# MasterXiong/Hyper-VLA

Hardware: AMD Instinct MI355X
Metric: actions_per_sec (higher is better)
Workload: dtype f16; 1 GPU; BASELINE configs[1]: hypernet weight-gen once (untimed) + full sample_actions step (u8 224x224 -> DINOv2-base E=768 in the loop -> generated vit_t 4L/64d policy -> [4,7] action chunk); 1 action = 1 sample-step; batch_per_gpu=256, global_batch=256, encoder=DINOv2-base (reference parity, E=768), parallelism=episode-dp1 (no collectives), policy_operands=split-bf16 (bf16x3), launch=eager (114 launches per step, counted by the library), streams=1, ensemble=not in the step

## Files before the change

hyper-vla_amd/csrc/api.hip:

```cpp
#include <hip/hip_runtime.h>

#include <cmath>
#include <cstdio>
#include <cstring>
#include <map>
#include <memory>
#include <mutex>
#include <string>
#include <vector>

#include "../../include/hvla.h"
#include "common.h"
#include "kernels.h"
#include "layout.h"
#include "pack.h"
#include "t5.h"
#include "train.h"

using namespace hvla;

namespace {

struct DevBuf {
  void* p = nullptr;
// ... 23 lines not shown
  int B = 0, H = 0;
  DevBuf ring;
  DevBuf state;
};

struct hvla_ctx {
  hvla_config cfg{};
  Geom g{};
  int device = 0;
  std::string err;
  bool loaded = false;
  bool train_timer = false;
  PackedLayout lay;
  int Kp = 0;
  DevBuf hn_f32;
  CtxParams ctxp{};
  DevBuf wcat_hi, wcat_lo, bcat, perm;
  DevBuf enc16, encd16, encf32;
  EncWeights encw{};
  DevBuf ctx_hi, ctx_lo, ctx_f32, ws_x, ws_h, ws_qkv, ws_g, ws_corr, ws_abar, ws_lncnt, ws_lnpart, tokens, flags;
  uint32_t ln_spin = 800;
#ifdef HVLA_BENCH_HOOKS
  int enc_stop = 0;
#endif
  Profiler prof;
  float *amap_dino = nullptr, *amap_head = nullptr;
  hipStream_t side = nullptr;
  hipEvent_t ev_fork = nullptr, ev_join = nullptr;
  std::vector<hvla_weights*> arena_pool;
  std::mutex pool_mu;
  static constexpr size_t ARENA_POOL_MAX = 4;
  hipEvent_t ev_bucket[3] = {nullptr, nullptr, nullptr};
  bool bucket_recorded[3] = {false, false, false};
  ~hvla_ctx() {
    for (hvla_weights* w : arena_pool) delete w;
    for (hipEvent_t e : ev_bucket)
      if (e) (void)hipEventDestroy(e);
    if (ev_fork) (void)hipEventDestroy(ev_fork);
    if (ev_join) (void)hipEventDestroy(ev_join);
    if (side) (void)hipStreamDestroy(side);
  }
  int rs_H = 0, rs_W = 0, rs_row_span = 0, rs_col_span = 0;
  DevBuf rs_tab, rs_rows, rs_img, rs_pad;
  bool t5_loaded = false;
  T5Dims t5d{};
  T5Weights t5w{};
// ... 406 lines not shown
  return HVLA_OK;
}

static int check_step(hvla_ctx* ctx, int32_t B) {
  if (!ctx->loaded) FAIL(ctx, HVLA_E_STATE, "called before hvla_load_weights");
  if (B < 1 || B > ctx->cfg.max_batch) FAIL(ctx, HVLA_E_SHAPE, "batch %d outside [1, %d]", B, ctx->cfg.max_batch);
  return HVLA_OK;
}

static int encode_range(hvla_ctx* ctx, const uint8_t* images, float* out, int b0, int nb, bool keep_cls, hipStream_t st) {
  const Geom& g = ctx->g;
  const size_t S = g.S(), E = g.E, F = g.enc_mlp, rows = (size_t)b0 * S;
  const size_t gper = S * F > (size_t)g.P() * ctx->Kp ? S * F : (size_t)g.P() * ctx->Kp;
  EncWorkspace ws{ctx->ws_x.as<float>() + rows * E, static_cast<char*>(ctx->ws_h.p) + rows * E * 2,
                  static_cast<char*>(ctx->ws_qkv.p) + rows * 3 * E * 2, static_cast<char*>(ctx->ws_g.p) + (size_t)b0 * gper * 2,
                  ctx->ws_corr.as<float>() + (size_t)2 * b0 * (F > 3 * E ? F : 3 * E),
                  static_cast<char*>(ctx->ws_abar.p) + (size_t)2 * b0 * (F > E ? F : E) * 2};
  if (ctx->amap_dino) ws.amap = ctx->amap_dino + (size_t)b0 * g.enc_layers * g.enc_heads * g.P();
  ws.ln_cnt = ctx->ws_lncnt.as<uint32_t>() + (size_t)((b0 + 3) / 4 * 4);
  ws.ln_part = ctx->ws_lnpart.as<float>() + (size_t)b0 * 4 * 256 * 4;
  ws.ln_spin = ctx->ln_spin;
#ifdef HVLA_BENCH_HOOKS
  ws.stop_after = ctx->enc_stop;
#endif
  const size_t img = (size_t)g.image_size * g.image_size * 3, per = (keep_cls ? S : (size_t)g.P()) * E;
  HIPCHK(ctx, launch_encoder(g, ctx->cfg.enc_dtype, ctx->encw, ws, images + (size_t)b0 * img, out + (size_t)b0 * per, nb, st,
                             &ctx->prof, keep_cls));
  return HVLA_OK;
}

int hvla_encode(hvla_ctx* ctx, const uint8_t* images, float* tokens, int32_t B, void* stream) {
  if (!ctx) return HVLA_E_STATE;
  if (int r = check_step(ctx, B)) return r;
  if (!images || !tokens) FAIL(ctx, HVLA_E_SHAPE, "null pointer");
  HIPCHK(ctx, hipSetDevice(ctx->device));
  return encode_range(ctx, images, tokens, 0, B, false, reinterpret_cast<hipStream_t>(stream));
}

int hvla_encode_hidden(hvla_ctx* ctx, const uint8_t* images, float* hidden, int32_t B, void* stream) {
  if (!ctx) return HVLA_E_STATE;
  if (int r = check_step(ctx, B)) return r;
  if (!images || !hidden) FAIL(ctx, HVLA_E_SHAPE, "null pointer");
  HIPCHK(ctx, hipSetDevice(ctx->device));
  return encode_range(ctx, images, hidden, 0, B, true, reinterpret_cast<hipStream_t>(stream));
}

// ... 619 lines not shown
  if (!ctx || !ptr || !bytes) return HVLA_E_STATE;
  DevBuf* b[8] = {&ctx->ws_x, &ctx->ws_h, &ctx->ws_qkv, &ctx->ws_g, &ctx->ws_corr, &ctx->ws_abar, &ctx->ws_lncnt, &ctx->ws_lnpart};
  if (which < 0 || which > 7) return HVLA_E_SHAPE;
  *ptr = b[which]->p;
  *bytes = b[which]->bytes;
  return HVLA_OK;
}
int hvla_debug_lnx_stats(hvla_ctx* ctx, unsigned long long* out, int reset) {
  if (!ctx) return HVLA_E_STATE;
  HIPCHK(ctx, hipSetDevice(ctx->device));
  HIPCHK(ctx, debug_lnx_stats(out, reset));
  return HVLA_OK;
}
int hvla_debug_encode_stop(hvla_ctx* ctx, int32_t n) {
  if (!ctx || n < 0) return HVLA_E_STATE;
  ctx->enc_stop = n;
  return HVLA_OK;
}
int hvla_debug_lnx_spin(hvla_ctx* ctx, uint32_t ticks) {
  if (!ctx) return HVLA_E_STATE;
  ctx->ln_spin = ticks;
  return HVLA_OK;
}
#endif

int64_t hvla_launches(hvla_ctx* ctx) {
  if (!ctx) return 0;
  const int64_t n = (int64_t)ctx->prof.nlaunch;
  ctx->prof.nlaunch = 0;
  return n;
}

int hvla_box_probe(hvla_ctx* ctx, float out[3], void* stream) {
  if (!ctx || !out) return HVLA_E_STATE;
  HIPCHK(ctx, hipSetDevice(ctx->device));
  DevBuf sink, ticks;
  int ncu = 256;
  (void)hipDeviceGetAttribute(&ncu, hipDeviceAttributeMultiprocessorCount, ctx->device);
  if (sink.alloc((size_t)ncu * 512 * sizeof(float)) != hipSuccess || ticks.alloc(64) != hipSuccess) FAIL(ctx, HVLA_E_ARENA_FULL, "box probe buffers");
  HIPCHK(ctx, run_box_probe(sink.as<float>(), ticks.as<unsigned long long>(), out, reinterpret_cast<hipStream_t>(stream)));
  return HVLA_OK;
}

int hvla_selftest(hvla_ctx* ctx, void* stream) {
  if (!ctx) return HVLA_E_STATE;
  HIPCHK(ctx, hipSetDevice(ctx->device));
// ... 13 lines not shown
```

hyper-vla_amd/csrc/encoder.hip:

```cpp
#include <cstring>
#include <type_traits>

#include "common.h"
#include "kernels.h"
#include "plan.h"

namespace hvla {

template <typename Op>
__global__ void im2col_kernel(const uint8_t* __restrict__ img, typename Op::elem* __restrict__ out, int B,
                              int image, int patch, int grid, int Kp, float* __restrict__ x, const float* __restrict__ pos, int S, int E) {
  for (size_t i = (size_t)blockIdx.x * blockDim.x + threadIdx.x; i < (size_t)B * E; i += (size_t)gridDim.x * blockDim.x)
    x[(i / E) * S * E + (i % E)] = pos[i % E];
  const int Kp1 = Kp / 2, chunks = Kp1 / 8;
  const size_t total = (size_t)B * grid * grid * chunks;
  const int kreal = patch * patch * 3;
  for (size_t i = (size_t)blockIdx.x * blockDim.x + threadIdx.x; i < total; i += (size_t)gridDim.x * blockDim.x) {
    const int ch = (int)(i % chunks);
    const size_t m = i / chunks;
    const int px = (int)(m % grid), py = (int)((m / grid) % grid);
    const size_t b = m / ((size_t)grid * grid);
    typename Op::x8 v;
    const int rowb = 3 * patch;
    const int k0 = ch * 8;
// ... 779 lines not shown
    reinterpret_cast<f32x4*>(partial + ((size_t)b * LNG + grp) * E)[threadIdx.x] = cs;
  }
}
template <typename Op>
__global__ __launch_bounds__(256) void layernorm_mean_kernel(const float* __restrict__ partial, typename Op::elem* __restrict__ abar,
                                                             int P, int E) {
  const int bh = blockIdx.x, n4 = E / 4;
  if ((int)threadIdx.x >= n4) return;
  const f32x4 t = ln_half_sum(reinterpret_cast<const f32x4*>(partial + (size_t)bh * 4 * E) + threadIdx.x, n4);
  const float inv = 1.f / (float)(P / 2);
  typename Op::x4 o;
#pragma unroll
  for (int j = 0; j < 4; ++j) o[j] = (typename Op::elem)(t[j] * inv);
  reinterpret_cast<typename Op::x4*>(abar + (size_t)bh * E)[threadIdx.x] = o;
}
constexpr int HBM_ = 256, HBN_ = 256;
constexpr int PRO_DMA = 12, PRO_DMA_KT0 = 8;
template <int EPI> struct EpiVmem { static constexpr int min_ops = (EPI == EPI_RES || EPI == EPI_PATCH) ? 64 : 32; };

#ifdef HVLA_BENCH_HOOKS
__device__ unsigned long long g_lnx_dbg[8][256];
#endif
constexpr int LNX_STAT = 98304, LNX_MR = LNX_STAT + 8192, LNX_CTRL = LNX_MR + 2048;
typedef __attribute__((address_space(3))) char lds_char;
template <typename Op, int EPI, bool PERSIST, bool LNX = false, bool NTOUT = false>
__global__ __launch_bounds__(512) void gemm256p_kernel(GemmArgs g) {
  static_assert(!NTOUT || EPI != EPI_PATCH, "NTOUT: non-temporal stores of the 16-bit outputs (QKV, GELU) / loads of the residual rows (RES)");
  using T = typename Op::elem;
  using X8 = typename Op::x8;
  static_assert(!LNX || EPI == EPI_RES || EPI == EPI_PATCH, "the fused LayerNorm follows a GEMM that writes the residual stream");
  extern __shared__ __attribute__((aligned(16))) char smem[];
  const int tid = threadIdx.x, lane = tid & 63;
  const int wave = __builtin_amdgcn_readfirstlane(tid >> 6);
  const int wm = wave >> 2, wn = wave & 3;
  const int nbm = g.nbm, nbn = (g.N + HBN_ - 1) / HBN_;
  const int ntiles = nbm * nbn;
  const int GN = nbn % 4 == 0 ? 4 : (nbn % 3 == 0 ? 3 : (nbn % 2 == 0 ? 2 : 1));
  auto tile_origin = [&](int v, int& tm, int& n0) {
    const int q = ntiles / 8, r = ntiles % 8, xcd = v % 8;
    const int bid = (xcd < r ? xcd * (q + 1) : r * (q + 1) + (xcd - r) * q) + v / 8;
    constexpr int CH = 8;
    const int per_chunk = CH * nbn;
    const int chunk = bid / per_chunk, rc = bid % per_chunk;
    const int rows = (nbm - chunk * CH) < CH ? (nbm - chunk * CH) : CH;
    const int sc = rc / (rows * GN), r2 = rc % (rows * GN);
    tm = chunk * CH + r2 / GN;
// ... 29 lines not shown
  const int sch = ((lane & 7) ^ (lane >> 3)) * 8;
  const uint32_t lane_a = ((uint32_t)srow * (uint32_t)g.K + sch) * (uint32_t)sizeof(T);
  const uint32_t lane_w = ((uint32_t)(wperm(srow)) * (uint32_t)g.K + sch) * (uint32_t)sizeof(T);
  const uint32_t lds0 = (uint32_t)(uintptr_t)(__attribute__((address_space(3))) char*)smem;
  const T* abase = A + (size_t)m0 * g.K;
  const T* wbase = W + (size_t)n0 * g.K;
  int wn0 = n0;
  const int KT = g.K / 64;
  auto stage = [&](auto hc, int kt) {
    constexpr int h = decltype(hc)::value;
    const int buf = kt & 1;
#pragma unroll
    for (int u = 0; u < 2; ++u) {
      const int j = 2 * (h & 1) + u;
      const int jw = (h < 2 || wn0 + 64 * j < g.N) ? j : 0;
      const T* sb = (h < 2 ? abase : wbase) + ((size_t)jw * 64 * g.K + kt * 64);
      const uint32_t dst = lds0 + (uint32_t)(buf * 65536 + wave * 1024 + (h >> 1) * 32768 + j * 8192);
      const uint32_t vo = h < 2 ? lane_a : lane_w;
      uint32_t keep;
      asm volatile("s_mov_b32 %0, m0\n\ts_mov_b32 m0, %3\n\ts_nop 0\n\tglobal_load_lds_dwordx4 %1, %2\n\ts_mov_b32 m0, %0"
                   : "=&s"(keep) : "v"(vo), "s"(sb), "s"(dst));
    }
  };
  f32x4 acc[4][8];
  const int fr = lane & 15, fq = lane >> 4;
  const int sw0 = ((fq) ^ (fr & 7)) << 4, sw1 = ((fq + 4) ^ (fr & 7)) << 4;
  const int a_off = (wm * 128 + fr) * 128, w_off = 32768 + (wn * 64 + fr) * 128;
  X8 fa0[8], fa1[8], fw0[4], fw1[4];
  auto rd_a = [&](X8 (&f)[8], const char* lb, int ah) {
#pragma unroll
    for (int t = 0; t < 4; ++t) {
      f[2 * t] = *reinterpret_cast<const X8*>(lb + a_off + (4 * ah + t) * 2048 + sw0);
      f[2 * t + 1] = *reinterpret_cast<const X8*>(lb + a_off + (4 * ah + t) * 2048 + sw1);
    }
  };
  auto rd_w = [&](X8 (&f)[4], const char* lb, int wh) {
#pragma unroll
    for (int t = 0; t < 2; ++t) {
      f[2 * t] = *reinterpret_cast<const X8*>(lb + w_off + (2 * wh + t) * 2048 + sw0);
      f[2 * t + 1] = *reinterpret_cast<const X8*>(lb + w_off + (2 * wh + t) * 2048 + sw1);
    }
  };
  auto quad = [&](const X8 (&fa)[8], const X8 (&fw)[4], auto ahc, auto whc) {
    constexpr int ah = decltype(ahc)::value, wh = decltype(whc)::value;
#pragma unroll
    for (int kk = 0; kk < 2; ++kk)
#pragma unroll
      for (int mt = 0; mt < 4; ++mt)
#pragma unroll
        for (int nt = 0; nt < 2; ++nt)
          acc[2 * wh + nt][4 * ah + mt] = Op::mma16(fa[2 * mt + kk], fw[2 * nt + kk], acc[2 * wh + nt][4 * ah + mt]);
  };
  using H0 = std::integral_constant<int, 0>;
  using H1 = std::integral_constant<int, 1>;
  using H2 = std::integral_constant<int, 2>;
  using H3 = std::integral_constant<int, 3>;
#define HVLA_BAR() do { __builtin_amdgcn_sched_barrier(0); __builtin_amdgcn_s_barrier(); __builtin_amdgcn_sched_barrier(0); } while (0)
  stage(H0{}, 0); stage(H1{}, 0); stage(H2{}, 0); stage(H3{}, 0);
  if (KT > 1) {
    stage(H0{}, 1); stage(H1{}, 1);
    asm volatile("s_waitcnt vmcnt(4)" ::: "memory");
  } else {
    asm volatile("s_waitcnt vmcnt(0)" ::: "memory");
  }
  auto ktile = [&](int kt, auto s1c, auto s2c) {
    constexpr bool S1 = decltype(s1c)::value, S2 = decltype(s2c)::value;
    const char* lb = smem + (kt & 1) * 65536;
    rd_w(fw0, lb, 0);
    rd_a(fa0, lb, 0);
    if constexpr (S1) stage(H2{}, kt + 1);
    HVLA_BAR();
    asm volatile("s_waitcnt lgkmcnt(0)" ::: "memory");
    quad(fa0, fw0, H0{}, H0{});
    HVLA_BAR();
    rd_w(fw1, lb, 1);
    rd_a(fa1, lb, 1);
    if constexpr (S1) stage(H3{}, kt + 1);
    asm volatile("s_waitcnt lgkmcnt(0)" ::: "memory");
    HVLA_BAR();
    quad(fa0, fw1, H0{}, H1{});
    HVLA_BAR();
    if constexpr (S2) stage(H0{}, kt + 2);
    HVLA_BAR();
    quad(fa1, fw1, H1{}, H1{});
    HVLA_BAR();
    if constexpr (S2) stage(H1{}, kt + 2);
    if constexpr (S2) asm volatile("s_waitcnt vmcnt(4)" ::: "memory");
    else if constexpr (S1) asm volatile("s_waitcnt vmcnt(0)" ::: "memory");
    HVLA_BAR();
    quad(fa1, fw0, H1{}, H0{});
// ... 6 lines not shown
    for (int i = 0; i < 4; ++i)
#pragma unroll
      for (int j = 0; j < 8; ++j) acc[i][j] = f32x4{0.f, 0.f, 0.f, 0.f};
    HVLA_BAR();
    if (wm == 1) HVLA_BAR();
    {
      int kt = 0;
      for (; kt + 2 < KT; ++kt) ktile(kt, Yes{}, Yes{});
      if (kt + 1 < KT) { ktile(kt, Yes{}, No{}); ++kt; }
      ktile(kt, No{}, No{});
    }
    if (wm == 0) HVLA_BAR();
    if constexpr (LNX) {
#pragma unroll
      for (int i = 0; i < 4; ++i)
#pragma unroll
        for (int j = 0; j < 8; ++j) asm volatile("" : "+v"(acc[i][j]));
    }
    const int cm0 = m0, cn0 = n0, ctm = tm;
    bool more = false;
    const float* brow = (EPI != EPI_PATCH && g.corr) ? g.corr + ((size_t)ctm * 2 + wm) * g.N : g.bias;
    const bool wvalid = cn0 + wn * 64 < g.N;
    f32x4 pb4 = f32x4{0.f, 0.f, 0.f, 0.f}, pl4 = pb4;
    int lane_e = lane;
    if constexpr (LNX) asm volatile("v_mbcnt_lo_u32_b32 %0, -1, 0\n\tv_mbcnt_hi_u32_b32 %0, -1, %0" : "=v"(lane_e));
    const int fr_e = LNX ? (lane_e & 15) : fr;
    if (wvalid) {
      const uint32_t vcol = (uint32_t)(cn0 + wn * 64 + 4 * fr_e);
      pb4 = *reinterpret_cast<const f32x4*>(brow + vcol);
      pl4 = pb4;
      if constexpr (EPI == EPI_RES) pl4 = *reinterpret_cast<const f32x4*>(g.aux + vcol);
    }
    asm volatile("" : "+v"(pb4), "+v"(pl4));
    const bool clater = later;
    if constexpr (PERSIST) {
      vb += gridDim.x;
      more = vb < ntiles;
      if (more) {
        if constexpr (LNX) tile_origin_x(tm, n0, later);
        else tile_origin(vb, tm, n0);
        m0 = g.tile_row0 + tm * g.tile_stride;
        abase = A + (size_t)m0 * g.K;
        wbase = W + (size_t)n0 * g.K;
        wn0 = n0;
        __builtin_amdgcn_sched_barrier(0);
        stage(H0{}, 0); stage(H1{}, 0); stage(H2{}, 0); stage(H3{}, 0);
        stage(H0{}, 1); stage(H1{}, 1);
        __builtin_amdgcn_sched_barrier(0);
      }
    }
    if constexpr (LNX) {
    } else if (!wvalid) {
    } else if constexpr (EPI == EPI_GELU) {
      if (g.colmean) {
        typename Op::x4 csh;
#pragma unroll
        for (int c = 0; c < 4; ++c) csh[c] = (T)0.f;
        gemm_epilogue_rows_impl<Op, EPI, 8, true, false, true, false, NTOUT>(acc, g, cm0 + wm * 128, cn0 + wn * 64, fr, fq, &pb4, &pl4, &csh);
        typename Op::x4 mo;
#pragma unroll
        for (int c = 0; c < 4; ++c) {
          float cs = (float)csh[c];
          cs += __shfl_xor(cs, 16, 64);
          cs += __shfl_xor(cs, 32, 64);
          mo[c] = (T)(cs * (1.f / 128.f));
        }
        if (fq == 0) *reinterpret_cast<typename Op::x4*>(reinterpret_cast<T*>(g.colmean) + ((size_t)ctm * 2 + wm) * g.N + cn0 + wn * 64 + 4 * fr) = mo;
      } else {
        gemm_epilogue_rows_impl<Op, EPI, 8, true, false, false, false, NTOUT>(acc, g, cm0 + wm * 128, cn0 + wn * 64, fr, fq, &pb4, &pl4);
      }
    } else {
      gemm_epilogue_rows_impl<Op, EPI, 8, true, false, false, false, NTOUT>(acc, g, cm0 + wm * 128, cn0 + wn * 64, fr, fq, &pb4, &pl4);
    }
    if constexpr (LNX) {
      typedef __attribute__((address_space(3))) float lds_f;
      typedef __attribute__((address_space(3))) f32x4 lds_f4;
      typedef __attribute__((address_space(3))) uint32_t lds_u;
      uint32_t lds_x = LNX_STAT;
      int nbn_x = nbn, wm_x = wm, wn_x = wn;
      asm volatile("" : "+s"(lds_x), "+s"(nbn_x), "+s"(wm_x), "+s"(wn_x));
      lds_f* stat = (lds_f*)((lds_char*)smem + lds_x);
      lds_f* mr = (lds_f*)((lds_char*)smem + lds_x + (LNX_MR - LNX_STAT));
      volatile lds_u* ctrl = (volatile lds_u*)((lds_char*)smem + lds_x + (LNX_CTRL - LNX_STAT));
      const int img = ctm, ct = cn0 / HBN_;
      typedef const __attribute__((address_space(4))) GemmArgs* karg_ptr;
      karg_ptr gp = (karg_ptr)__builtin_amdgcn_kernarg_segment_ptr();
      asm volatile("" : "+s"(gp));
      int tid_x = wave * 64 + lane_e;
      asm volatile("" : "+v"(tid_x));
      const int lane_x = tid_x & 63, fr_x = lane_x & 15, fq_x = lane_x >> 4;
      const uint32_t row0 = (uint32_t)(img * gp->S + 1 + wm_x * 128 + 4 * fq_x);
      uint32_t pend_old = 0;
      if constexpr (PERSIST) {
        if (pend_img >= 0 && tid_x == 0)
          pend_old = __hip_atomic_fetch_add(gp->ln_cnt + pend_img, 1u + pend_mark, __ATOMIC_RELAXED, __HIP_MEMORY_SCOPE_AGENT);
      }
      const float invE = 1.f / (float)gp->N;
#ifdef HVLA_BENCH_HOOKS
      const unsigned long long dbg_t0 = __builtin_readcyclecounter();
      unsigned long long dbg_wait = 0;
#endif
#define HVLA_LBAR() do { asm volatile("s_waitcnt lgkmcnt(0)" ::: "memory"); __builtin_amdgcn_s_barrier(); asm volatile("" ::: "memory"); } while (0)
      const __amdgpu_buffer_rsrc_t xrs = __builtin_amdgcn_make_buffer_rsrc(gp->out, 0, (int)gp->out_bytes, 0x00020000);
      const uint32_t lane_el = row0 * (uint32_t)gp->N + (uint32_t)(wn_x * 64 + 4 * fr_x);
      f32x4 xk[8][4];
      {
        __amdgpu_buffer_rsrc_t irs = xrs;
        uint32_t ivo = (lane_el + (uint32_t)cn0) * 4u;
        if constexpr (EPI == EPI_PATCH) {
          irs = __builtin_amdgcn_make_buffer_rsrc(const_cast<float*>(gp->aux), 0, gp->S * gp->N * 4, 0x00020000);
          ivo = ((uint32_t)(1 + wm_x * 128 + 4 * fq_x) * (uint32_t)gp->N + (uint32_t)(cn0 + wn_x * 64 + 4 * fr_x)) * 4u;
        }
        const float q = gp->qscale;
        const float vmask = wvalid ? 1.f : 0.f;
        constexpr int XR = 3;
        f32x4 xin[XR][4];
        int rowb = gp->N * 4;
        asm volatile("" : "+s"(rowb));
        auto request = [&](int mt) {
#pragma unroll
          for (int r = 0; r < 4; ++r)
            xin[mt % XR][r] = __builtin_bit_cast(f32x4, __builtin_amdgcn_raw_buffer_load_b128(irs, (int)ivo, (16 * mt + r) * rowb, (EPI == EPI_RES && NTOUT) ? 2 : 0));
        };
#pragma unroll
        for (int mt = 0; mt < XR - 1; ++mt) request(mt);
#pragma unroll
        for (int mt = 0; mt < 8; ++mt) {
          if (mt + XR - 1 < 8) request(mt + XR - 1);
          f32x4 t[4];
#pragma unroll
          for (int c = 0; c < 4; ++c) {
            if constexpr (EPI == EPI_PATCH) t[c] = __builtin_elementwise_fma(acc[c][mt], f32x4{q, q, q, q}, f32x4{pb4[c], pb4[c], pb4[c], pb4[c]});
            else t[c] = acc[c][mt] + pb4[c];
          }
#pragma unroll
          for (int r = 0; r < 4; ++r) {
            f32x4 x = xin[mt % XR][r];
#pragma unroll
            for (int c = 0; c < 4; ++c) {
              if constexpr (EPI == EPI_RES) x[c] = fmaf(t[c][r], pl4[c], x[c]);
              else x[c] += t[c][r];
            }
            xk[mt][r] = x;
            asm volatile("" : "+v"(xk[mt][r]));
          }
          {
            float sv[4], qv[4];
#pragma unroll
            for (int r = 0; r < 4; ++r) {
              ln_lane_stats(xk[mt][r], sv[r], qv[r]);
              sv[r] = row16_sum(sv[r]) * vmask;
              qv[r] = row16_sum(qv[r]) * vmask;
            }
            if (fr_x == 0) {
              lds_f4* d = (lds_f4*)(stat + (wn_x * 256 + wm_x * 128 + 16 * mt + 4 * fq_x) * 2);
              d[0] = f32x4{sv[0], qv[0], sv[1], qv[1]};
              d[1] = f32x4{sv[2], qv[2], sv[3], qv[3]};
            }
          }
          __builtin_amdgcn_sched_barrier(0);
        }
      }
#ifdef HVLA_BENCH_HOOKS
      const unsigned long long dbg_tA = __builtin_readcyclecounter();
#endif
      HVLA_LBAR();
      typedef float f2 __attribute__((ext_vector_type(2)));
      const __amdgpu_buffer_rsrc_t prs = __builtin_amdgcn_make_buffer_rsrc(gp->ln_part, 0, (int)gp->part_bytes, 0x00020000);
      const uint32_t tag = gp->ln_tag;
      auto ent = [](u32x4 e) { const f32x4 f = __builtin_bit_cast(f32x4, e); return f2{f[0], f[2]}; };
      const int prow = tid_x & 255;
      f2 mine;
      {
        typedef __attribute__((address_space(3))) f2 lds_f2;
        const f2 p0 = *(lds_f2*)(stat + (0 * 256 + prow) * 2), p1 = *(lds_f2*)(stat + (1 * 256 + prow) * 2);
        const f2 p2 = *(lds_f2*)(stat + (2 * 256 + prow) * 2), p3 = *(lds_f2*)(stat + (3 * 256 + prow) * 2);
        mine = (p0 + p1) + (p2 + p3);
      }
      if (tid_x < 256) {
        const float tagf = __builtin_bit_cast(float, tag);
        const f32x4 ef = f32x4{mine[0], tagf, mine[1], tagf};
        __builtin_amdgcn_raw_buffer_store_b128(__builtin_bit_cast(u32x4, ef), prs, (int)((uint32_t)((img * nbn_x + ct) * 256 + prow) * 16u), 0, 16);
      }
      f32x4 lg4 = f32x4{0.f, 0.f, 0.f, 0.f}, lb4 = lg4;
      if (wvalid) {
        const uint32_t vcol = (uint32_t)(cn0 + wn_x * 64 + 4 * fr_x);
        lg4 = *reinterpret_cast<const f32x4*>(gp->ln_scale + vcol);
        lb4 = *reinterpret_cast<const f32x4*>(gp->ln_bias + vcol);
      }
      const __amdgpu_buffer_rsrc_t hrs = __builtin_amdgcn_make_buffer_rsrc(gp->ln_out, 0, (int)(gp->out_bytes / 4u * (uint32_t)sizeof(T)), 0x00020000);
      auto store_x = [&]() {
        if (!wvalid) return;
        const uint32_t vo = (lane_el + (uint32_t)cn0) * 4u;
        int rowb = gp->N * 4;
        asm volatile("" : "+s"(rowb));
#pragma unroll
        for (int mt = 0; mt < 8; ++mt)
#pragma unroll
          for (int r = 0; r < 4; ++r)
            __builtin_amdgcn_raw_buffer_store_b128(__builtin_bit_cast(u32x4, xk[mt][r]), xrs, (int)vo, (16 * mt + r) * rowb,
                                                   (NTOUT ? 18 : 16));
      };
#ifdef HVLA_BENCH_HOOKS
      const unsigned long long dbg_tB = __builtin_readcyclecounter();
#endif
      if (wave >= 4) {
        bool ok = !clater;
        f2 t = mine;
        if (ok) {
          const uint64_t t0 = __builtin_amdgcn_s_memrealtime();
          const uint32_t eo = (uint32_t)(img * nbn_x * 256 + prow) * 16u;
          while (true) {
            u32x4 pe[4];
#pragma unroll
            for (int c = 0; c < 4; ++c)
              if (c < nbn_x) pe[c] = __builtin_amdgcn_raw_buffer_load_b128(prs, (int)eo, c * 4096, 16);
            ok = true;
#pragma unroll
            for (int c = 0; c < 4; ++c)
              if (c < nbn_x && c != ct) ok = ok && pe[c][1] == tag && pe[c][3] == tag;
            if (__builtin_amdgcn_ballot_w64(ok) == ~0ull) {
              f2 pv[4];
#pragma unroll
              for (int c = 0; c < 4; ++c) pv[c] = c == ct ? mine : ent(pe[c]);
              t = pv[0];
#pragma unroll
              for (int c = 1; c < 4; ++c)
                if (c < nbn_x) t += pv[c];
              break;
            }
            if (__builtin_amdgcn_s_memrealtime() - t0 > (uint64_t)gp->ln_spin) break;
            __builtin_amdgcn_s_sleep(1);
          }
        }
        const bool wave_ok = __builtin_amdgcn_ballot_w64(ok) == ~0ull;
        if (wave_ok) {
// ... 59 lines not shown
          }
          __builtin_amdgcn_sched_barrier(0);
        }
        if (gp->ln_abar) {
          typename Op::x4 mo;
#pragma unroll
          for (int c = 0; c < 4; ++c) {
            float t = cs[c];
            t = xor32_sum(xor16_sum(t));
            mo[c] = (T)(t * (1.f / 128.f));
          }
          if (fq_x == 0) *reinterpret_cast<typename Op::x4*>(reinterpret_cast<T*>(gp->ln_abar) + ((size_t)im * 2 + wm_x) * gp->N + ncol) = mo;
        }
      };
      if (go && wvalid) sweep(img, ct, lg4, lb4);
      auto from_memory = [&](int im, uint32_t bits) {
        if (wave == 0) {
          __builtin_amdgcn_fence(__ATOMIC_ACQUIRE, "agent");
          asm volatile("s_waitcnt vmcnt(0)" ::: "memory");
        }
        HVLA_LBAR();
        if (tid_x < 256) {
          const uint32_t eo = (uint32_t)(im * nbn_x * 256 + tid_x) * 16u;
          u32x4 pe[4];
#pragma unroll
          for (int c = 0; c < 4; ++c)
            if (c < nbn_x) pe[c] = __builtin_amdgcn_raw_buffer_load_b128(prs, (int)eo, c * 4096, 0);
          f2 t = ent(pe[0]);
#pragma unroll
          for (int c = 1; c < 4; ++c)
            if (c < nbn_x) t += ent(pe[c]);
          float mean, rstd;
          ln_finish(t[0], t[1], invE, mean, rstd);
          *(__attribute__((address_space(3))) f2*)(mr + tid_x * 2) = f2{mean, rstd};
        }
        HVLA_LBAR();
        for (int c = 0; c < nbn_x; ++c) {
          if (!((bits >> (16 + c)) & 1u) || c * HBN_ + wn_x * 64 >= gp->N) continue;
          const uint32_t ncol = (uint32_t)(c * HBN_ + wn_x * 64 + 4 * fr_x);
          const f32x4 gm4 = *reinterpret_cast<const f32x4*>(gp->ln_scale + ncol), bt4 = *reinterpret_cast<const f32x4*>(gp->ln_bias + ncol);
          {
            const uint32_t vox = ((uint32_t)(im * gp->S + 1 + wm_x * 128 + 4 * fq_x) * (uint32_t)gp->N + ncol) * 4u;
            const uint32_t voh = ((uint32_t)(im * gp->S + 1 + wm_x * 128 + 4 * fq_x) * (uint32_t)gp->N + ncol) * (uint32_t)sizeof(T);
            int rowbx = gp->N * 4, rowbh = gp->N * (int)sizeof(T);
            asm volatile("" : "+s"(rowbx), "+s"(rowbh));
            f32x4 ring[3][4];
            auto req = [&](int mt) {
// ... 59 lines not shown
        pend_mark = my_mark;
      }
      if (!PERSIST || !more) {
        asm volatile("s_waitcnt vmcnt(0)" ::: "memory");
        HVLA_LBAR();
        uint32_t old = 0;
        if (tid_x == 0) old = __hip_atomic_fetch_add(gp->ln_cnt + img, 1u + my_mark, __ATOMIC_RELAXED, __HIP_MEMORY_SCOPE_AGENT);
        settle(img, my_mark, old);
      }
#ifdef HVLA_BENCH_HOOKS
      if (tid_x == 0 && blockIdx.x < 256) {
        atomicAdd(&g_lnx_dbg[0][blockIdx.x], 1ull);
        atomicAdd(&g_lnx_dbg[1][blockIdx.x], (unsigned long long)__builtin_readcyclecounter() - dbg_t0);
        atomicAdd(&g_lnx_dbg[2][blockIdx.x], dbg_wait);
        if (!go) atomicAdd(&g_lnx_dbg[3][blockIdx.x], 1ull);
        if (dbg_slow) atomicAdd(&g_lnx_dbg[4][blockIdx.x], dbg_slow);
        atomicAdd(&g_lnx_dbg[5][blockIdx.x], dbg_tA - dbg_t0);
        atomicAdd(&g_lnx_dbg[6][blockIdx.x], dbg_tB - dbg_tA);
        atomicAdd(&g_lnx_dbg[7][blockIdx.x], (unsigned long long)__builtin_readcyclecounter() - dbg_tC);
      }
#endif
#undef HVLA_LBAR
      if (!more) break;
      if (wvalid) asm volatile("s_waitcnt vmcnt(63)" ::: "memory");
      else asm volatile("s_waitcnt vmcnt(0)" ::: "memory");
      continue;
    }
    if (!more) break;
    constexpr int WAITN = (PRO_DMA - PRO_DMA_KT0) + EpiVmem<EPI>::min_ops;
    static_assert(EpiVmem<EPI>::min_ops >= 32, "an epilogue issues at least one store per row of the wave tile");
    static_assert(WAITN >= 63 || WAITN == 36, "the s_waitcnt immediates below are written for these two counts");
    if (!wvalid) asm volatile("s_waitcnt vmcnt(%0)" ::"n"(PRO_DMA - PRO_DMA_KT0) : "memory");
    else if constexpr (WAITN >= 63) asm volatile("s_waitcnt vmcnt(63)" ::: "memory");
    else asm volatile("s_waitcnt vmcnt(36)" ::: "memory");
  }
#undef HVLA_BAR
}

template <typename Op, int FINAL>
__global__ __launch_bounds__(256) void layernorm_kernel(const float* __restrict__ x, void* __restrict__ out,
                                                        const float* __restrict__ scale,
                                                        const float* __restrict__ bias, int M, int E, int S) {
  const int row = blockIdx.x * 4 + (threadIdx.x >> 6), lane = threadIdx.x & 63;
  if (row >= M) return;
  if (FINAL == 1 && (row % S) == 0) return;
  const f32x4* xr = reinterpret_cast<const f32x4*>(x + (size_t)row * E);
  const int n4 = E / 4;
// ... 587 lines not shown
    SETA((gemm64c_kernel<Op, EPI_QKV>)) SETA((gemm64c_kernel<Op, EPI_GELU>)) SETA((gemm64c_kernel<Op, EPI_RES>)) SETA((gemm64c32_kernel<Op>))
    SETA((gemm64c_kernel<Op, EPI_QKV, true>)) SETA((gemm64c_kernel<Op, EPI_GELU, true>)) SETA((layernorm_group_kernel<Op>))
    SETA((gemm256p_kernel<Op, EPI_QKV, false, false, true>)) SETA((gemm256p_kernel<Op, EPI_GELU, false, false, true>))
    SETA((gemm256p_kernel<Op, EPI_QKV, true, false, true>)) SETA((gemm256p_kernel<Op, EPI_GELU, true, false, true>))
    SETA((gemm256p_kernel<Op, EPI_RES, false, false, true>)) SETA((gemm256p_kernel<Op, EPI_RES, true, false, true>))
#undef SETA
    di.attr[opi] = true;
  }
  if (!di.ncu && (hipDeviceGetAttribute(&di.ncu, hipDeviceAttributeMultiprocessorCount, dev) != hipSuccess || di.ncu <= 0)) di.ncu = 256;
  const int ncu = di.ncu;
  constexpr int G64_MAXM = 2047;
  constexpr int CAT_COMP = 8;
  const bool comp = w.layer[0].dqkv != nullptr && ws.corr && ws.abar;
  const int hsplit = 1 + P / 2;
  bool ln_fused = false;
  uint32_t ln_launch = 0;
  auto small_fused = [&](int N, int K) {
    return comp && M <= G64_MAXM && (size_t)M * K < (1ull << 31) && (size_t)N * K < (1ull << 31) && N % SBN == 0 && K % 64 == 0 && S >= 9;
  };
  const float* ln_partial = nullptr;
  const bool can_fuse_ln = ws.ln_cnt != nullptr && ws.ln_part != nullptr && (size_t)M * E * 4 < (1ull << 32) && E <= 1024;
  auto lnx_persistent = [&](int nbm_, int nbn_) {
    const int nt = nbm_ * nbn_;
    if (ncu % 8 || nt % ncu || nbm_ % 8) return false;
    const int Wx = ncu / 8, odd = Wx % nbn_, R = nt / ncu;
    return Wx >= nbn_ && (odd == 0 || R % nbn_ == 0);
  };
  auto lnx_args = [&](GemmArgs& a, const float* ln_s, const float* ln_b, int nbn_) {
    a.ln_out = ws.h; a.ln_scale = ln_s; a.ln_bias = ln_b; a.ln_abar = comp ? ws.abar : nullptr; a.ln_cnt = ws.ln_cnt; a.ln_part = ws.ln_part;
    a.out_bytes = (uint32_t)((size_t)M * E * 4);
    a.part_bytes = (uint32_t)((size_t)B * nbn_ * 256 * 16);
    a.ln_tag = ++ln_launch;
    a.ln_target = ln_launch * (uint32_t)nbn_;
    a.ln_spin = ws.ln_spin;
    if (lnx_persistent((int)a.nbm, nbn_)) {
      const int Wx = ncu / 8, R = a.nbm * nbn_ / ncu;
      a.lnx_G = Wx / nbn_; a.lnx_rows_aligned = R * a.lnx_G; a.lnx_rounds_div = R / nbn_; a.lnx_rows_xcd = a.nbm / 8;
      a.lnx_rcp = (65536 + nbn_ - 1) / nbn_;
    }
  };
  auto gemm = [&](auto epic, const void* A, const void* Wt, const void* dW, int N, int K, const float* bias, const float* aux,
                  void* out, int qcols, int cat, void* colmean = nullptr, const float* ln_s = nullptr, const float* ln_b = nullptr) -> bool {
    constexpr int EPI = decltype(epic)::value;
    ln_fused = false;
    GemmArgs a{A, Wt, M, N, K, bias, aux, out, P, S, qcols, qcols ? 0.125f * 1.4426950408889634f : 1.f / 256.f};
    a.hsplit = hsplit;
    const bool fits32 = (size_t)M * K < (1ull << 31) && (size_t)N * K < (1ull << 31);
    const bool aligned = P == HBM_ && N % SBN == 0 && N >= HBN_ && M > G64_MAXM && K >= 128 && K % 64 == 0 && fits32;
    if (aligned) {
      pf.begin(CAT_COMP, st);
      GemmArgs c = a;
      c.M = B; c.row0 = 0; c.row_step = S;
      int nblocks = ((B + SBM - 1) / SBM) * (N / SBN);
      if (comp) { c.abar2 = ws.abar; c.dW2 = dW; c.corr2 = ws.corr; c.M2 = 2 * B; nblocks += ((2 * B + SBM - 1) / SBM) * (N / SBN); }
      if constexpr (EPI != EPI_PATCH) {
        if (nblocks > ncu) HVLA_LAUNCH((gemm64_kernel<Op, EPI, 4>), dim3(nblocks), dim3(256), 4 * 16384, st, c);
        else HVLA_LAUNCH((gemm64_kernel<Op, EPI>), dim3(nblocks), dim3(256), SNS * 16384, st, c);
      } else {
        HVLA_LAUNCH((gemm64_kernel<Op, EPI>), dim3(nblocks), dim3(256), SNS * 16384, st, c);
      }
      pf.end(CAT_COMP, st);
      const int nbn = (N + HBN_ - 1) / HBN_;
      a.corr = comp ? ws.corr : nullptr;
      a.nbm = B; a.tile_row0 = 1; a.tile_stride = S; a.colmean = colmean;
      const size_t lds = 131072;
      pf.begin(cat, st);
      if constexpr (EPI == EPI_RES) {
        if (ln_s && can_fuse_ln) {
          lnx_args(a, ln_s, ln_b, nbn);
          const bool nt = big_output(M, N, sizeof(float));
          if (lnx_persistent(B, nbn)) {
            if (nt) HVLA_LAUNCH((gemm256p_kernel<Op, EPI, true, true, true>), dim3(ncu), dim3(512), lds, st, a);
            else HVLA_LAUNCH((gemm256p_kernel<Op, EPI, true, true>), dim3(ncu), dim3(512), lds, st, a);
          } else {
            if (nt) HVLA_LAUNCH((gemm256p_kernel<Op, EPI, false, true, true>), dim3(B * nbn), dim3(512), lds, st, a);
            else HVLA_LAUNCH((gemm256p_kernel<Op, EPI, false, true>), dim3(B * nbn), dim3(512), lds, st, a);
          }
          pf.end(cat, st);
          ln_fused = true;
          return true;
        }
      }
      if constexpr (EPI != EPI_PATCH) {
        if (big_output(M, N, EPI == EPI_RES ? sizeof(float) : sizeof(T)) && (EPI == EPI_RES || nt16_addressable(M, N, sizeof(T)))) {
          if ((B * nbn) % ncu == 0) HVLA_LAUNCH((gemm256p_kernel<Op, EPI, true, false, true>), dim3(ncu), dim3(512), lds, st, a);
          else HVLA_LAUNCH((gemm256p_kernel<Op, EPI, false, false, true>), dim3(B * nbn), dim3(512), lds, st, a);
          pf.end(cat, st);
          return true;
        }
      }
      if ((B * nbn) % ncu == 0) HVLA_LAUNCH((gemm256p_kernel<Op, EPI, true>), dim3(ncu), dim3(512), lds, st, a);
      else HVLA_LAUNCH((gemm256p_kernel<Op, EPI, false>), dim3(B * nbn), dim3(512), lds, st, a);
      pf.end(cat, st);
      return true;
    }
    if constexpr (EPI != EPI_PATCH) {
      if (small_fused(N, K)) {
        a.abar2 = ws.abar; a.dW2 = dW; a.M2 = 2 * B;
        pf.begin(cat, st);
// ... 59 lines not shown
    if ((e = hipMemsetAsync(ws.ln_cnt, 0, (size_t)((B * 4 + 15) / 16 * 16), st)) != hipSuccess) return e;
    if ((e = hipMemsetAsync(ws.ln_part, 0, (size_t)B * ((E + HBN_ - 1) / HBN_) * 256 * 16, st)) != hipSuccess) return e;
    pf.nlaunch += 2;
  }
  using EQ = std::integral_constant<int, EPI_QKV>;
  using EG = std::integral_constant<int, EPI_GELU>;
  using ER = std::integral_constant<int, EPI_RES>;
  pf.begin(0, st);
  {
    const size_t total = (size_t)B * P * (Kp / 16);
    int blocks = (int)((total + 255) / 256);
    if (blocks > 8192) blocks = 8192;
    HVLA_LAUNCH(im2col_kernel<Op>, dim3(blocks), dim3(256), 0, st, images, reinterpret_cast<T*>(ws.g), B,
                       g.image_size, g.patch, g.grid(), Kp, ws.x, w.pos, S, E);
    const int Mp = B * P;
    GemmArgs a{ws.g, w.w_patch, Mp, E, Kp, w.b_patch, w.pos, ws.x, P, S, 0, 1.f / 256.f};
    const bool fits32 = (size_t)Mp * Kp < (1ull << 31);
    if (Mp % HBM_ == 0 && E % SBN == 0 && E >= HBN_ && Mp > G64_MAXM && fits32) {
      a.nbm = Mp / HBM_; a.tile_row0 = 0; a.tile_stride = HBM_;
      const int nbn = (E + HBN_ - 1) / HBN_;
      if (P == HBM_ && can_fuse_ln && g.enc_layers > 0) {
        a.hsplit = hsplit;
        lnx_args(a, w.layer[0].ln1_s, w.layer[0].ln1_b, nbn);
        if (lnx_persistent(a.nbm, nbn)) HVLA_LAUNCH((gemm256p_kernel<Op, EPI_PATCH, true, true>), dim3(ncu), dim3(512), 131072, st, a);
        else HVLA_LAUNCH((gemm256p_kernel<Op, EPI_PATCH, false, true>), dim3(a.nbm * nbn), dim3(512), 131072, st, a);
        ln_fused = true;
      } else if ((a.nbm * nbn) % ncu == 0) HVLA_LAUNCH((gemm256p_kernel<Op, EPI_PATCH, true>), dim3(ncu), dim3(512), 131072, st, a);
      else HVLA_LAUNCH((gemm256p_kernel<Op, EPI_PATCH, false>), dim3(a.nbm * nbn), dim3(512), 131072, st, a);
    } else if (Mp <= G64_MAXM && fits32 && E % SBN == 0) {
      HVLA_LAUNCH((gemm64_kernel<Op, EPI_PATCH>), dim3(((Mp + SBM - 1) / SBM) * (E / SBN)), dim3(256), SNS * 16384, st, a);
    } else {
      HVLA_LAUNCH((gemm_kernel<Op, EPI_PATCH>), dim3(((Mp + GBM - 1) / GBM) * (E / GBN)), dim3(256), gsm, st, a);
    }
  }
  pf.end(0, st);
  const int KT = (S + 31) / 32;
  const size_t asm_bytes = (size_t)KT * 32 * 2 * AVLD * sizeof(T) + (size_t)KT * APS * sizeof(float) + 64 * sizeof(T) +
                           (size_t)(KT - 1) * 64 * sizeof(float);
#ifdef HVLA_BENCH_HOOKS
  int products = 0;
#define HVLA_STOP_HERE() do { if (ws.stop_after > 0 && ++products == ws.stop_after) return hipGetLastError(); } while (0)
#else
#define HVLA_STOP_HERE() do { } while (0)
#endif
  for (int l = 0; l < g.enc_layers; ++l) {
    const EncLayerW& L = w.layer[l];
    if (!ln_fused) {
      pf.begin(1, st);
// ... 134 lines not shown
```

hyper-vla_amd/csrc/kernels.h:

```cpp
#pragma once
#include <hip/hip_runtime.h>
#include <stdint.h>

#include <vector>

#include "../../include/hvla.h"
#include "layout.h"

namespace hvla {

struct CtxLayer {
  const float *ln0_s, *ln0_b, *wq, *bq, *wk, *bk, *wv, *bv, *wo, *bo, *ln1_s, *ln1_b, *w1, *b1, *w2, *b2;
};
constexpr int CTX_MAX_LAYERS = 8;
struct CtxParams {
  int T, C, F, heads, layers, lang_dim, E, scale_context;
  int big_elems;
  const float* tok;
  const int64_t* attn_mask;
  const float* cls;
  const float *w_tok, *b_tok, *w_img, *b_img, *pos_tok, *pos_img, *pos_layer, *norm_s, *norm_b;
  CtxLayer layer[CTX_MAX_LAYERS];
  float* ctx;
  __bf16 *ctx_hi, *ctx_lo;
// ... 22 lines not shown
  const float *ln1_s, *ln1_b, *ln2_s, *ln2_b, *ls1, *ls2;
};
constexpr int ENC_MAX_LAYERS = 24;
struct EncWeights {
  const void* w_patch;
  const float* b_patch;
  const float* pos;
  const float *lnf_s, *lnf_b;
  EncLayerW layer[ENC_MAX_LAYERS];
};
struct EncWorkspace {
  float* x;
  void* h;
  void* qkv;
  void* g;
  float* corr;
  void* abar;
  float* amap = nullptr;
  uint32_t* ln_cnt = nullptr;
  float* ln_part = nullptr;
  uint32_t ln_spin = 800;
#ifdef HVLA_BENCH_HOOKS
  int stop_after = 0;
#endif
};
struct Profiler {
  int mode = 0;
  uint32_t select = 1u << 5;
  std::vector<hipEvent_t> start, stop;
  std::vector<int> cat;
  size_t used = 0;
  uint64_t nlaunch = 0;
  bool want(int c) const { return c >= 0 && (mode == 2 || (mode == 1 && ((select >> c) & 1u))); }
  void begin(int c, hipStream_t st) {
    if (!want(c)) return;
    if (used == start.size()) {
      hipEvent_t a, b;
      if (hipEventCreate(&a) != hipSuccess || hipEventCreate(&b) != hipSuccess) return;
      start.push_back(a), stop.push_back(b), cat.push_back(c);
    }
    cat[used] = c;
    (void)hipEventRecord(start[used], st);
  }
  void end(int c, hipStream_t st) {
    if (!want(c) || used >= start.size()) return;
    (void)hipEventRecord(stop[used], st);
// ... 82 lines not shown
```

Measured before the change: 18200 actions/s.

## Prefetch residual rows into LDS via async DMA during fused-LN GEMM tail

In the fused GEMM+LayerNorm (LNX) kernel, the residual/patch rows are now fetched with global_load_lds DMA into extra LDS slots. The first three m-tiles are issued during the last k-tiles, replacing the register-based buffer loads issued only after the GEMM finished. The bias and LN vectors are loaded unconditionally with inline asm. The next tile's prologue staging is moved after the LN barrier so it overlaps the cross-block statistics wait. LDS use grows to 160KB, which may lower occupancy, and the hand-written vmcnt counting is fragile. Debug hooks for forcing the non-persistent path and borrowing the x buffer are also added.

```diff
diff --git a/hyper-vla_amd/csrc/api.hip b/hyper-vla_amd/csrc/api.hip
--- a/hyper-vla_amd/csrc/api.hip
+++ b/hyper-vla_amd/csrc/api.hip
@@ -69,6 +69,7 @@
   uint32_t ln_spin = 800;
 #ifdef HVLA_BENCH_HOOKS
   int enc_stop = 0;
+  int lnx_one_tile = 0;
 #endif
   Profiler prof;
   float *amap_dino = nullptr, *amap_head = nullptr;
@@ -521,6 +522,7 @@
   ws.ln_spin = ctx->ln_spin;
 #ifdef HVLA_BENCH_HOOKS
   ws.stop_after = ctx->enc_stop;
+  ws.lnx_one_tile = ctx->lnx_one_tile;
 #endif
   const size_t img = (size_t)g.image_size * g.image_size * 3, per = (keep_cls ? S : (size_t)g.P()) * E;
   HIPCHK(ctx, launch_encoder(g, ctx->cfg.enc_dtype, ctx->encw, ws, images + (size_t)b0 * img, out + (size_t)b0 * per, nb, st,
@@ -1186,6 +1188,25 @@
   ctx->ln_spin = ticks;
   return HVLA_OK;
 }
+int hvla_debug_lnx_one_tile(hvla_ctx* ctx, int32_t on) {
+  if (!ctx) return HVLA_E_STATE;
+  ctx->lnx_one_tile = on;
+  return HVLA_OK;
+}
+int hvla_debug_borrow_x(hvla_ctx* ctx, void* ptr, size_t bytes) {
+  static void* own_p = nullptr;
+  static size_t own_bytes = 0;
+  if (!ctx) return HVLA_E_STATE;
+  if (ptr) {
+    if (own_p) return HVLA_E_STATE;
+    own_p = ctx->ws_x.p; own_bytes = ctx->ws_x.bytes;
+    ctx->ws_x.p = ptr; ctx->ws_x.bytes = bytes;
+  } else if (own_p) {
+    ctx->ws_x.p = own_p; ctx->ws_x.bytes = own_bytes;
+    own_p = nullptr;
+  }
+  return HVLA_OK;
+}
 #endif
 
 int64_t hvla_launches(hvla_ctx* ctx) {
diff --git a/hyper-vla_amd/csrc/encoder.hip b/hyper-vla_amd/csrc/encoder.hip
--- a/hyper-vla_amd/csrc/encoder.hip
+++ b/hyper-vla_amd/csrc/encoder.hip
@@ -825,6 +825,8 @@
 __device__ unsigned long long g_lnx_dbg[8][256];
 #endif
 constexpr int LNX_STAT = 98304, LNX_MR = LNX_STAT + 8192, LNX_CTRL = LNX_MR + 2048;
+constexpr int LNX_XSLOT0 = 131072, LNX_LDS = 163840;
+__device__ __forceinline__ constexpr int lnx_xslot(int mt) { return (mt & 3) == 0 ? LNX_XSLOT0 : ((mt & 3) - 1) * 32768; }
 typedef __attribute__((address_space(3))) char lds_char;
 template <typename Op, int EPI, bool PERSIST, bool LNX = false, bool NTOUT = false>
 __global__ __launch_bounds__(512) void gemm256p_kernel(GemmArgs g) {
@@ -900,6 +902,38 @@
                    : "=&s"(keep) : "v"(vo), "s"(sb), "s"(dst));
     }
   };
+  struct XSrc { const float* sb; uint32_t vo, dst, rowb; };
+  auto xsrc = [&](int tmv, int n0v, int wmv, int wnv) {
+    typedef const __attribute__((address_space(4))) GemmArgs* karg_ptr;
+    karg_ptr ga = (karg_ptr)__builtin_amdgcn_kernarg_segment_ptr();
+    asm volatile("" : "+s"(ga));
+    int lx;
+    asm volatile("v_mbcnt_lo_u32_b32 %0, -1, 0\n\tv_mbcnt_hi_u32_b32 %0, -1, %0" : "=v"(lx));
+    const int Nn = ga->N;
+    const int wne = n0v + wnv * 64 < Nn ? wnv : 0;
+    const float* src = EPI == EPI_PATCH ? ga->aux : reinterpret_cast<const float*>(ga->out);
+    const uint32_t row = (EPI == EPI_PATCH ? 0u : (uint32_t)(tmv * ga->S)) + (uint32_t)(1 + wmv * 128);
+    XSrc x;
+    x.sb = src + ((size_t)row * (uint32_t)Nn + (uint32_t)(n0v + wne * 64));
+    x.vo = ((uint32_t)(lx >> 4) * 4u * (uint32_t)Nn + 4u * (uint32_t)(lx & 15)) * 4u;
+    x.dst = lds0 + (uint32_t)((wmv * 4 + wnv) * 4096);
+    x.rowb = (uint32_t)Nn * 4u;
+    return x;
+  };
+  auto xdma = [&](int mt, const XSrc& x) {
+#pragma unroll
+    for (int r = 0; r < 4; ++r) {
+      const float* sr = reinterpret_cast<const float*>(reinterpret_cast<const char*>(x.sb) + (size_t)(16 * mt + r) * x.rowb);
+      const uint32_t d = x.dst + (uint32_t)(lnx_xslot(mt) + r * 1024);
+      uint32_t keep;
+      if constexpr (EPI == EPI_RES && NTOUT)
+        asm volatile("s_mov_b32 %0, m0\n\ts_mov_b32 m0, %3\n\ts_nop 2\n\tglobal_load_lds_dwordx4 %1, %2 nt ; lnx-x-dma\n\ts_mov_b32 m0, %0"
+                     : "=&s"(keep) : "v"(x.vo), "s"(sr), "s"(d));
+      else
+        asm volatile("s_mov_b32 %0, m0\n\ts_mov_b32 m0, %3\n\ts_nop 2\n\tglobal_load_lds_dwordx4 %1, %2 ; lnx-x-dma\n\ts_mov_b32 m0, %0"
+                     : "=&s"(keep) : "v"(x.vo), "s"(sr), "s"(d));
+    }
+  };
   f32x4 acc[4][8];
   const int fr = lane & 15, fq = lane >> 4;
   const int sw0 = ((fq) ^ (fr & 7)) << 4, sw1 = ((fq + 4) ^ (fr & 7)) << 4;
@@ -943,7 +977,9 @@
   }
   auto ktile = [&](int kt, auto s1c, auto s2c) {
     constexpr bool S1 = decltype(s1c)::value, S2 = decltype(s2c)::value;
+    constexpr bool XL = LNX && !S1 && !S2;
     const char* lb = smem + (kt & 1) * 65536;
+    if constexpr (XL) { const XSrc x = xsrc(tm, n0, wm, wn); xdma(0, x); xdma(1, x); xdma(2, x); }
     rd_w(fw0, lb, 0);
     rd_a(fa0, lb, 0);
     if constexpr (S1) stage(H2{}, kt + 1);
@@ -996,9 +1032,15 @@
     const float* brow = (EPI != EPI_PATCH && g.corr) ? g.corr + ((size_t)ctm * 2 + wm) * g.N : g.bias;
     const bool wvalid = cn0 + wn * 64 < g.N;
     f32x4 pb4 = f32x4{0.f, 0.f, 0.f, 0.f}, pl4 = pb4;
+    uint32_t pend_old = 0;
     int lane_e = lane;
     if constexpr (LNX) asm volatile("v_mbcnt_lo_u32_b32 %0, -1, 0\n\tv_mbcnt_hi_u32_b32 %0, -1, %0" : "=v"(lane_e));
     const int fr_e = LNX ? (lane_e & 15) : fr;
+    if constexpr (LNX) {
+      const uint32_t vcolb = (uint32_t)(cn0 + (wvalid ? wn : 0) * 64 + 4 * fr_e) * 4u;
+      asm volatile("s_nop 4\n\tglobal_load_dwordx4 %0, %1, %2" : "=v"(pb4) : "v"(vcolb), "s"(brow));
+      if constexpr (EPI == EPI_RES) asm volatile("s_nop 4\n\tglobal_load_dwordx4 %0, %1, %2" : "=v"(pl4) : "v"(vcolb), "s"(g.aux));
+    } else {
     if (wvalid) {
       const uint32_t vcol = (uint32_t)(cn0 + wn * 64 + 4 * fr_e);
       pb4 = *reinterpret_cast<const f32x4*>(brow + vcol);
@@ -1006,6 +1048,7 @@
       if constexpr (EPI == EPI_RES) pl4 = *reinterpret_cast<const f32x4*>(g.aux + vcol);
     }
     asm volatile("" : "+v"(pb4), "+v"(pl4));
+    }
     const bool clater = later;
     if constexpr (PERSIST) {
       vb += gridDim.x;
@@ -1017,10 +1060,12 @@
         abase = A + (size_t)m0 * g.K;
         wbase = W + (size_t)n0 * g.K;
         wn0 = n0;
-        __builtin_amdgcn_sched_barrier(0);
-        stage(H0{}, 0); stage(H1{}, 0); stage(H2{}, 0); stage(H3{}, 0);
-        stage(H0{}, 1); stage(H1{}, 1);
-        __builtin_amdgcn_sched_barrier(0);
+        if constexpr (!LNX) {
+          __builtin_amdgcn_sched_barrier(0);
+          stage(H0{}, 0); stage(H1{}, 0); stage(H2{}, 0); stage(H3{}, 0);
+          stage(H0{}, 1); stage(H1{}, 1);
+          __builtin_amdgcn_sched_barrier(0);
+        }
       }
     }
     if constexpr (LNX) {
@@ -1063,44 +1108,35 @@
       int tid_x = wave * 64 + lane_e;
       asm volatile("" : "+v"(tid_x));
       const int lane_x = tid_x & 63, fr_x = lane_x & 15, fq_x = lane_x >> 4;
-      const uint32_t row0 = (uint32_t)(img * gp->S + 1 + wm_x * 128 + 4 * fq_x);
-      uint32_t pend_old = 0;
-      if constexpr (PERSIST) {
-        if (pend_img >= 0 && tid_x == 0)
-          pend_old = __hip_atomic_fetch_add(gp->ln_cnt + pend_img, 1u + pend_mark, __ATOMIC_RELAXED, __HIP_MEMORY_SCOPE_AGENT);
-      }
       const float invE = 1.f / (float)gp->N;
 #ifdef HVLA_BENCH_HOOKS
       const unsigned long long dbg_t0 = __builtin_readcyclecounter();
       unsigned long long dbg_wait = 0;
 #endif
 #define HVLA_LBAR() do { asm volatile("s_waitcnt lgkmcnt(0)" ::: "memory"); __builtin_amdgcn_s_barrier(); asm volatile("" ::: "memory"); } while (0)
-      const __amdgpu_buffer_rsrc_t xrs = __builtin_amdgcn_make_buffer_rsrc(gp->out, 0, (int)gp->out_bytes, 0x00020000);
-      const uint32_t lane_el = row0 * (uint32_t)gp->N + (uint32_t)(wn_x * 64 + 4 * fr_x);
       f32x4 xk[8][4];
       {
-        __amdgpu_buffer_rsrc_t irs = xrs;
-        uint32_t ivo = (lane_el + (uint32_t)cn0) * 4u;
-        if constexpr (EPI == EPI_PATCH) {
-          irs = __builtin_amdgcn_make_buffer_rsrc(const_cast<float*>(gp->aux), 0, gp->S * gp->N * 4, 0x00020000);
-          ivo = ((uint32_t)(1 + wm_x * 128 + 4 * fq_x) * (uint32_t)gp->N + (uint32_t)(cn0 + wn_x * 64 + 4 * fr_x)) * 4u;
-        }
         const float q = gp->qscale;
         const float vmask = wvalid ? 1.f : 0.f;
-        constexpr int XR = 3;
-        f32x4 xin[XR][4];
-        int rowb = gp->N * 4;
-        asm volatile("" : "+s"(rowb));
-        auto request = [&](int mt) {
-#pragma unroll
-          for (int r = 0; r < 4; ++r)
-            xin[mt % XR][r] = __builtin_bit_cast(f32x4, __builtin_amdgcn_raw_buffer_load_b128(irs, (int)ivo, (16 * mt + r) * rowb, (EPI == EPI_RES && NTOUT) ? 2 : 0));
-        };
-#pragma unroll
-        for (int mt = 0; mt < XR - 1; ++mt) request(mt);
+        const XSrc xe_src = xsrc(ctm, cn0, wm_x, wn_x);
+        xdma(3, xe_src);
+        const uint32_t xoff = (uint32_t)((tid_x >> 6) * 4096 + lane_x * 16);
+        if constexpr (EPI != EPI_RES) asm volatile("s_waitcnt vmcnt(4) ; lnx-x-ready" : "+v"(pb4) :: "memory");
+        else asm volatile("s_waitcnt vmcnt(4) ; lnx-x-ready" : "+v"(pb4), "+v"(pl4) :: "memory");
+        if constexpr (EPI != EPI_RES) pl4 = pb4;
 #pragma unroll
         for (int mt = 0; mt < 8; ++mt) {
-          if (mt + XR - 1 < 8) request(mt + XR - 1);
+          if (mt == 3 || mt == 4) asm volatile("s_waitcnt vmcnt(12)" ::: "memory");
+          if (mt == 5) asm volatile("s_waitcnt vmcnt(8)" ::: "memory");
+          if (mt == 6) asm volatile("s_waitcnt vmcnt(4)" ::: "memory");
+          if (mt == 7) asm volatile("s_waitcnt vmcnt(0)" : "+v"(pend_old) :: "memory");
+          if constexpr (PERSIST) {
+            if (mt == 3 && pend_img >= 0 && tid_x == 0)
+              asm volatile("s_nop 4\n\tglobal_atomic_add %0, %1, %2, %3 sc0" : "=v"(pend_old) : "v"((uint32_t)pend_img * 4u), "v"(1u + pend_mark), "s"(gp->ln_cnt));
+          }
+          f32x4 xs[4];
+#pragma unroll
+          for (int r = 0; r < 4; ++r) xs[r] = *(const lds_f4*)((lds_char*)smem + xoff + (uint32_t)(lnx_xslot(mt) + r * 1024));
           f32x4 t[4];
 #pragma unroll
           for (int c = 0; c < 4; ++c) {
@@ -1109,7 +1145,7 @@
           }
 #pragma unroll
           for (int r = 0; r < 4; ++r) {
-            f32x4 x = xin[mt % XR][r];
+            f32x4 x = xs[r];
 #pragma unroll
             for (int c = 0; c < 4; ++c) {
               if constexpr (EPI == EPI_RES) x[c] = fmaf(t[c][r], pl4[c], x[c]);
@@ -1132,6 +1168,7 @@
               d[1] = f32x4{sv[2], qv[2], sv[3], qv[3]};
             }
           }
+          if (mt + 4 < 8) xdma(mt + 4, xe_src);
           __builtin_amdgcn_sched_barrier(0);
         }
       }
@@ -1139,7 +1176,18 @@
       const unsigned long long dbg_tA = __builtin_readcyclecounter();
 #endif
       HVLA_LBAR();
+      if constexpr (PERSIST) {
+        if (more) {
+          __builtin_amdgcn_sched_barrier(0);
+          stage(H0{}, 0); stage(H1{}, 0); stage(H2{}, 0); stage(H3{}, 0);
+          stage(H0{}, 1); stage(H1{}, 1);
+          __builtin_amdgcn_sched_barrier(0);
+        }
+      }
       typedef float f2 __attribute__((ext_vector_type(2)));
+      const uint32_t row0 = (uint32_t)(img * gp->S + 1 + wm_x * 128 + 4 * fq_x);
+      const __amdgpu_buffer_rsrc_t xrs = __builtin_amdgcn_make_buffer_rsrc(gp->out, 0, (int)gp->out_bytes, 0x00020000);
+      const uint32_t lane_el = row0 * (uint32_t)gp->N + (uint32_t)(wn_x * 64 + 4 * fr_x);
       const __amdgpu_buffer_rsrc_t prs = __builtin_amdgcn_make_buffer_rsrc(gp->ln_part, 0, (int)gp->part_bytes, 0x00020000);
       const uint32_t tag = gp->ln_tag;
       auto ent = [](u32x4 e) { const f32x4 f = __builtin_bit_cast(f32x4, e); return f2{f[0], f[2]}; };
@@ -1185,7 +1233,7 @@
           const uint64_t t0 = __builtin_amdgcn_s_memrealtime();
           const uint32_t eo = (uint32_t)(img * nbn_x * 256 + prow) * 16u;
           while (true) {
-            u32x4 pe[4];
+            u32x4 pe[4] = {};
 #pragma unroll
             for (int c = 0; c < 4; ++c)
               if (c < nbn_x) pe[c] = __builtin_amdgcn_raw_buffer_load_b128(prs, (int)eo, c * 4096, 16);
@@ -1291,7 +1339,7 @@
         HVLA_LBAR();
         if (tid_x < 256) {
           const uint32_t eo = (uint32_t)(im * nbn_x * 256 + tid_x) * 16u;
-          u32x4 pe[4];
+          u32x4 pe[4] = {};
 #pragma unroll
           for (int c = 0; c < 4; ++c)
             if (c < nbn_x) pe[c] = __builtin_amdgcn_raw_buffer_load_b128(prs, (int)eo, c * 4096, 0);
@@ -1397,7 +1445,8 @@
 #endif
 #undef HVLA_LBAR
       if (!more) break;
-      if (wvalid) asm volatile("s_waitcnt vmcnt(63)" ::: "memory");
+      if (wvalid && go) asm volatile("s_waitcnt vmcnt(63)" ::: "memory");
+      else if (wvalid) asm volatile("s_waitcnt vmcnt(%0)" ::"n"(PRO_DMA - PRO_DMA_KT0 + 32) : "memory");
       else asm volatile("s_waitcnt vmcnt(0)" ::: "memory");
       continue;
     }
@@ -2031,6 +2080,9 @@
   const bool can_fuse_ln = ws.ln_cnt != nullptr && ws.ln_part != nullptr && (size_t)M * E * 4 < (1ull << 32) && E <= 1024;
   auto lnx_persistent = [&](int nbm_, int nbn_) {
     const int nt = nbm_ * nbn_;
+#ifdef HVLA_BENCH_HOOKS
+    if (ws.lnx_one_tile) return false;
+#endif
     if (ncu % 8 || nt % ncu || nbm_ % 8) return false;
     const int Wx = ncu / 8, odd = Wx % nbn_, R = nt / ncu;
     return Wx >= nbn_ && (odd == 0 || R % nbn_ == 0);
@@ -2072,18 +2124,18 @@
       const int nbn = (N + HBN_ - 1) / HBN_;
       a.corr = comp ? ws.corr : nullptr;
       a.nbm = B; a.tile_row0 = 1; a.tile_stride = S; a.colmean = colmean;
-      const size_t lds = 131072;
+      const size_t lds = 131072, lds_lnx = LNX_LDS;
       pf.begin(cat, st);
       if constexpr (EPI == EPI_RES) {
-        if (ln_s && can_fuse_ln) {
+        if (ln_s && can_fuse_ln && K % 128 == 0) {
           lnx_args(a, ln_s, ln_b, nbn);
           const bool nt = big_output(M, N, sizeof(float));
           if (lnx_persistent(B, nbn)) {
-            if (nt) HVLA_LAUNCH((gemm256p_kernel<Op, EPI, true, true, true>), dim3(ncu), dim3(512), lds, st, a);
-            else HVLA_LAUNCH((gemm256p_kernel<Op, EPI, true, true>), dim3(ncu), dim3(512), lds, st, a);
+            if (nt) HVLA_LAUNCH((gemm256p_kernel<Op, EPI, true, true, true>), dim3(ncu), dim3(512), lds_lnx, st, a);
+            else HVLA_LAUNCH((gemm256p_kernel<Op, EPI, true, true>), dim3(ncu), dim3(512), lds_lnx, st, a);
           } else {
-            if (nt) HVLA_LAUNCH((gemm256p_kernel<Op, EPI, false, true, true>), dim3(B * nbn), dim3(512), lds, st, a);
-            else HVLA_LAUNCH((gemm256p_kernel<Op, EPI, false, true>), dim3(B * nbn), dim3(512), lds, st, a);
+            if (nt) HVLA_LAUNCH((gemm256p_kernel<Op, EPI, false, true, true>), dim3(B * nbn), dim3(512), lds_lnx, st, a);
+            else HVLA_LAUNCH((gemm256p_kernel<Op, EPI, false, true>), dim3(B * nbn), dim3(512), lds_lnx, st, a);
           }
           pf.end(cat, st);
           ln_fused = true;
@@ -2189,8 +2241,8 @@
       if (P == HBM_ && can_fuse_ln && g.enc_layers > 0) {
         a.hsplit = hsplit;
         lnx_args(a, w.layer[0].ln1_s, w.layer[0].ln1_b, nbn);
-        if (lnx_persistent(a.nbm, nbn)) HVLA_LAUNCH((gemm256p_kernel<Op, EPI_PATCH, true, true>), dim3(ncu), dim3(512), 131072, st, a);
-        else HVLA_LAUNCH((gemm256p_kernel<Op, EPI_PATCH, false, true>), dim3(a.nbm * nbn), dim3(512), 131072, st, a);
+        if (lnx_persistent(a.nbm, nbn)) HVLA_LAUNCH((gemm256p_kernel<Op, EPI_PATCH, true, true>), dim3(ncu), dim3(512), LNX_LDS, st, a);
+        else HVLA_LAUNCH((gemm256p_kernel<Op, EPI_PATCH, false, true>), dim3(a.nbm * nbn), dim3(512), LNX_LDS, st, a);
         ln_fused = true;
       } else if ((a.nbm * nbn) % ncu == 0) HVLA_LAUNCH((gemm256p_kernel<Op, EPI_PATCH, true>), dim3(ncu), dim3(512), 131072, st, a);
       else HVLA_LAUNCH((gemm256p_kernel<Op, EPI_PATCH, false>), dim3(a.nbm * nbn), dim3(512), 131072, st, a);
diff --git a/hyper-vla_amd/csrc/kernels.h b/hyper-vla_amd/csrc/kernels.h
--- a/hyper-vla_amd/csrc/kernels.h
+++ b/hyper-vla_amd/csrc/kernels.h
@@ -68,6 +68,7 @@
   uint32_t ln_spin = 800;
 #ifdef HVLA_BENCH_HOOKS
   int stop_after = 0;
+  int lnx_one_tile = 0;
 #endif
 };
 struct Profiler {
```

New measurement: 18380 actions/s, median of 6. About the same (+1.0%).
